# facebook/facebook360_dep

Measured on AMD Instinct MI355X. Metric: depth Mpix/s per GPU (full pyramid, 16-cam 2048^2 rig); % HBM-read roofline, higher is better.
Workload: dtype f32+f64; 1 GPU; BASELINE config 3: 16-camera 2048x2048 synthetic rig, 8-frame sequence, full 10-level pyramid per frame, per-level temporal filter (+-2 frames); the same sequence for every --gpus N (block partition, 8 frame(s) on this rank); rig=cfg2, cameras=16, frames=8, temporal_filter=True, halo_transport=local, parallelism=frames x1

## Files before the change

### facebook360_dep_amd/csrc/derp_capi.hip

```cpp
#include <hip/hip_runtime.h>

#include <algorithm>
#include <cmath>
#include <cstdarg>
#include <cstdio>
#include <cstdlib>
#include <cstring>
#include <map>
#include <memory>
#include <string>
#include <vector>

#include "../../include/derp_hip.h"
#include "derp_kernels.h"
#include "derp_points.h"
#include "derp_render.h"

using namespace derp;

namespace {

enum Stage {
  ST_FOV = 0,
  ST_VARIANCE,
// ... 1794 lines not shown
    return fail(c, "bad arguments");
  }
  const int L = c->cur;
  const size_t n = npx(c, L);
  TRY(upload_tmp(c, c->w.staging, disp, n));
  ALLOC(c, c->w.stagingB, 2 * n * sizeof(float));
  HIPCHK(c, hipMemsetAsync(c->w.stagingB.p, 0xff, 2 * n * sizeof(float), c->stream));
  LevelView V = make_view(c, ST_PINGPONG, 0, c->D);
  int tilesX;
  const int tiles = tiles_of(V.W, V.H, tilesX);
  const size_t lds = kCostLdsPerSrc * (size_t)(c->S);
  hipLaunchKernelGGL(k_cost_map, dim3(tiles), dim3(kCostBlock), lds, c->stream, V, d, c->w.staging.as<float>(),
                     c->w.stagingB.as<float>(), c->w.stagingB.as<float>() + n, tilesX);
  KCHECK(c);
  HIPCHK(c, hipStreamSynchronize(c->stream));
  HIPCHK(c, hipMemcpy(cost, c->w.stagingB.p, n * sizeof(float), hipMemcpyDeviceToHost));
  HIPCHK(c, hipMemcpy(confidence, c->w.stagingB.as<float>() + n, n * sizeof(float), hipMemcpyDeviceToHost));
  return 0;
}

int derp_debug_atan2_ypos(derp_ctx* c, const double* y, const double* x, double* out, size_t n) {
  if (!c || !y || !x || !out) {
    return fail(c, "bad arguments");
  }
  ALLOC(c, c->w.staging, 3 * n * sizeof(double));
  double* d = c->w.staging.as<double>();
  HIPCHK(c, hipMemcpyAsync(d, y, n * sizeof(double), hipMemcpyHostToDevice, c->stream));
  HIPCHK(c, hipMemcpyAsync(d + n, x, n * sizeof(double), hipMemcpyHostToDevice, c->stream));
  hipLaunchKernelGGL(k_debug_atan2_ypos, dim3(flat_grid(n)), dim3(256), 0, c->stream, d, d + n, d + 2 * n, n);
  KCHECK(c);
  HIPCHK(c, hipMemcpyAsync(out, d + 2 * n, n * sizeof(double), hipMemcpyDeviceToHost, c->stream));
  HIPCHK(c, hipStreamSynchronize(c->stream));
  return 0;
}

int derp_debug_fp64(derp_ctx* c, int op, const double* a, const double* b, double* out, size_t n) {
  if (!c || !a || !out || op < 0 || op > 3 || (op >= 2 && !b)) {
    return fail(c, "bad arguments");
  }
  if (n == 0) {
    return 0;
  }
  ALLOC(c, c->w.staging, 3 * n * sizeof(double));
  double* d = c->w.staging.as<double>();
  HIPCHK(c, hipMemcpyAsync(d, a, n * sizeof(double), hipMemcpyHostToDevice, c->stream));
  HIPCHK(c, hipMemcpyAsync(d + n, op >= 2 ? b : a, n * sizeof(double), hipMemcpyHostToDevice, c->stream));
  hipLaunchKernelGGL(k_debug_fp64, dim3(flat_grid(n)), dim3(256), 0, c->stream, op, d, d + n, d + 2 * n, n);
  KCHECK(c);
  HIPCHK(c, hipMemcpyAsync(out, d + 2 * n, n * sizeof(double), hipMemcpyDeviceToHost, c->stream));
  HIPCHK(c, hipStreamSynchronize(c->stream));
  return 0;
}

int derp_debug_sees(derp_ctx* c, int src, const double* xyz, size_t n, double* out) {
  if (!c || !xyz || !out || src < 0 || src >= c->S) {
    return fail(c, "bad arguments");
  }
  if (n == 0) {
    return 0;
  }
  ALLOC(c, c->w.staging, 9 * n * sizeof(double));
  double* d = c->w.staging.as<double>();
  HIPCHK(c, hipMemcpyAsync(d, xyz, 3 * n * sizeof(double), hipMemcpyHostToDevice, c->stream));
  hipLaunchKernelGGL(k_debug_sees, dim3(flat_grid(n)), dim3(256), 0, c->stream, c->camsSrc.as<Cam>(), src, d, d + 3 * n, n);
  KCHECK(c);
  HIPCHK(c, hipMemcpyAsync(out, d + 3 * n, 6 * n * sizeof(double), hipMemcpyDeviceToHost, c->stream));
  HIPCHK(c, hipStreamSynchronize(c->stream));
  return 0;
}

int derp_debug_download(derp_ctx* c, int d, int s, int which, void* out) {
  TRY(need_current(c, false));
  const int L = c->cur;
  const int W = c->LW[L], H = c->LH[L];
  const size_t n = (size_t)W * H;
  HIPCHK(c, hipStreamSynchronize(c->stream));
  if (which == 4) {
    HIPCHK(c, hipMemcpy(out, c->w.srcVar.as<float>() + (size_t)s * n, n * sizeof(float), hipMemcpyDeviceToHost));
    return 0;
  }
  if (which == 5) {
    HIPCHK(c, hipMemcpy(out, c->w.fovMask.as<uint8_t>() + (size_t)d * n, n, hipMemcpyDeviceToHost));
    return 0;
  }
  if (d < 0 || d >= c->D || s < 0 || s >= c->S || s == c->dst2srcH[d]) {
    return fail(c, "bad (dst, src) pair");
  }
  const size_t tab = (size_t)d * (c->S - 1) + (s < c->dst2srcH[d] ? s : s - 1);
  if (which == 0) {
    const int PW = W + 2 * kPadW, PH = H + 2 * kPadW;
    std::vector<float2> tmp((size_t)PW * PH);
    HIPCHK(c, hipMemcpy(tmp.data(), c->projWarp.as<float2>() + tab * tmp.size(), tmp.size() * sizeof(float2),
                        hipMemcpyDeviceToHost));
    float2* o = reinterpret_cast<float2*>(out);
    for (int y = 0; y < H; ++y) {
      memcpy(o + (size_t)y * W, &tmp[(size_t)(y + kPadW) * PW + kPadW], (size_t)W * sizeof(float2));
    }
    return 0;
  }
  if (which == 2 || which == 3) {
    const int PW = W + 2 * kPadC, PH = H + 2 * kPadC;
    std::vector<ushort4> tmp((size_t)PW * PH);
    const ushort4* base = (which == 2 ? c->w.projColor.as<ushort4>() : c->w.projBias.as<ushort4>()) + tab * tmp.size();
    HIPCHK(c, hipMemcpy(tmp.data(), base, tmp.size() * sizeof(ushort4), hipMemcpyDeviceToHost));
    uint16_t* o = reinterpret_cast<uint16_t*>(out);
    for (int y = 0; y < H; ++y) {
// ... 1060 lines not shown
```

### facebook360_dep_amd/csrc/derp_kernels.h

```cpp
#pragma once
#include <hip/hip_runtime.h>
#include <math.h>
#include <stdint.h>

#include <type_traits>

#include "derp_camera.h"
#include "gcc_algos.h"

namespace derp {

#ifndef DERP_COST_MIN_WAVES
#define DERP_COST_MIN_WAVES 4
#endif
#ifndef DERP_RANDOM_MIN_WAVES
#define DERP_RANDOM_MIN_WAVES 4
#endif
#ifndef DERP_RANDOM_TILED
#define DERP_RANDOM_TILED 0
#endif
#ifndef DERP_MIX_HOT_ONLY
#define DERP_MIX_HOT_ONLY 0
#endif
#ifndef DERP_PHASE_TIMERS
// ... 602 lines not shown
      const Cam& cs = V.camsSrc[s];
      D2 pn;
      const bool vis = sees<cost_sees_lean<RANDOM>()>(cs, pWorld, cs.principal[0], cs.principal[1], cs.focal[0], cs.focal[1],
                                                      1.0, 1.0, pn, pairs.atanLut);
      if (__ballot(pend) != 0ull) {
        consume();
      }
      pend = vis;
      pendSlot = slot(s, own);
      if (__ballot(vis) != 0ull) {
        const float sx = (float)(pn.x * V.Wd), sy = (float)(pn.y * V.Hd);
        const float xf = roundf(sx), yf = roundf(sy);
        const int xi = (int)xf, yi = (int)yf;
        pxw = sx - xf + 0.5f;
        pyw = sy - yf + 0.5f;
        const size_t tab = (size_t)dl * (V.S - 1) + pendSlot;
        const char* wbase = reinterpret_cast<const char*>(V.projWarp + tab * wPlane);
        const unsigned woff = vis ? ((unsigned)(yi - 1 + kPadW) * (unsigned)wPitch + (unsigned)(xi - 1 + kPadW)) * 8u : 0u;
        pa = *reinterpret_cast<const f4a8*>(wbase + woff);
        pb = *reinterpret_cast<const f4a8*>(wbase + (woff + (unsigned)wPitch * 8u));
      }
    }
    if (__ballot(pend) != 0ull) {
      consume();
    }
  }
  const unsigned tc1 = phase_clock();
  const int ssdCount = __popc(mask);
  nPair += ssdCount;
#ifdef DERP_COUNT_UNION
  if (slots) {
    *slots += __popc(__builtin_amdgcn_readfirstlane(waveMask));
  }
#endif
  int keep = 1;
  if (ssdCount < keep) {
    return make_float2(3.402823466e+38f, 0.0f);
  }
  {
    int cnt = 0;
    for (unsigned wm = __builtin_amdgcn_readfirstlane(waveMask); wm != 0; wm &= wm - 1) {
      const int t = __builtin_ctz(wm);
      if ((mask >> t) & 1) {
        const SsdPair e = pairs.get(t);
        const SsdPair ssd = compute_ssd<RANDOM>(V, px, colBase + (size_t)t * cPlane, biaBase + (size_t)t * cPlane, e.first,
                                                        e.second, RANDOM ? colTBase + (size_t)t * tPlane : nullptr);
        pairs.set(cnt, ssd);
        ++cnt;
      }
    }
  }
  const unsigned tc2 = phase_clock();
  keep = max(keep, ssdCount - 2);
  GccSelect<LdsPairs> sel(pairs);
  sel.nth_element(keep, ssdCount);
  float cost = 0;
  for (int i = 0; i < keep; ++i) {
    cost += pairs.get(i).second;
  }
  cost /= (float)keep;
  const float trustCoef = 1.0f / (float)keep;
  float confidence = px.confidence;
  if constexpr (RELOAD_RAY) {
    unsigned i = pix;
    asm("" : "+v"(i) : "v"(cost));
    if constexpr (RANDOM) {
      confidence = fmaxf(at32(V.srcVar + (size_t)own * ((size_t)V.W * V.H), i), kMinVar);
    } else {
      confidence = fmaxf((V.srcVar + (size_t)own * ((size_t)V.W * V.H))[i], kMinVar);
    }
  }
  const float costFinal = cost * trustCoef / confidence;
#if DERP_PHASE_TIMERS
  if (tm) {
    const unsigned tc3 = phase_clock();
    tm->proj += tc1 - tc0, tm->ssd += tc2 - tc1, tm->select += tc3 - tc2, tm->inside += tc3 - tc0;
  }
#endif
  return make_float2(costFinal, confidence);
}

template <bool WITH_RAY = true>
__device__ __forceinline__ void load_pixctx(const LevelView& V, int d, int own, int x, int y, const PatchWin* win, PixCtx& px,
                                            int tl = -1) {
  const Cam& cd = V.camsDst[d];
  px.rayO = {cd.pos[0], cd.pos[1], cd.pos[2]};
  const size_t n = (size_t)V.W * V.H;
  if constexpr (!WITH_RAY) {
    px.rayD = {0, 0, 0};
  } else {
    const size_t i = (size_t)d * n + (size_t)y * V.W + x;
    px.rayD = {V.rayDir[i], V.rayDir[V.rayStride + i], V.rayDir[2 * V.rayStride + i]};
  }
  if (tl < 0) {
    tl = (int)(threadIdx.x & 63);
  }
  const int corner = (tl >> 3) * kWinW + (tl & 7);
  px.winBG = win->bg + corner;
  px.winR = win->r + corner;
  const ushort4 b = V.ownBias[(size_t)own * n + (size_t)y * V.W + x];
  px.dstBiasBG = (v2f){(float)b.x, (float)b.y};
  px.dstBiasR = (float)b.z;
  const float var = V.srcVar[(size_t)own * n + (size_t)y * V.W + x];
  px.confidence = fmaxf(var, kMinVar);
}

__device__ __forceinline__ void flush_counters(const LevelView& V, unsigned nCost, unsigned nPair) {
  for (int off = 32; off > 0; off >>= 1) {
    nCost += __shfl_down(nCost, off);
    nPair += __shfl_down(nPair, off);
  }
  if ((threadIdx.x & 63) == 0) {
    atomicAdd(&V.counters[0], (unsigned long long)nCost);
    atomicAdd(&V.counters[1], (unsigned long long)nPair);
  }
}

__global__ void k_bgr_to_bgrx(const uint16_t* __restrict__ in, ushort4* __restrict__ out, size_t n) {
  size_t i = (size_t)blockIdx.x * blockDim.x + threadIdx.x;
  const size_t step = (size_t)gridDim.x * blockDim.x;
  for (; i < n; i += step) {
    out[i] = make_ushort4(in[3 * i], in[3 * i + 1], in[3 * i + 2], 0);
  }
}

__global__ void k_debug_atan2_ypos(const double* __restrict__ y, const double* __restrict__ x, double* __restrict__ out,
                                   size_t n) {
  size_t i = (size_t)blockIdx.x * blockDim.x + threadIdx.x;
  const size_t step = (size_t)gridDim.x * blockDim.x;
#if defined(__HIP_DEVICE_COMPILE__)
  __shared__ double atanLut[kAtanLutDoubles];
  atan_lut_fill(atanLut);
  __syncthreads();
  for (; i < n; i += step) {
    const double a = atan2_ypos(y[i], x[i]);
    const double b = atan2_ypos_lut(y[i], x[i], atanLut);
    out[i] = (__double_as_longlong(a) == __double_as_longlong(b)) ? b : __builtin_nan("");
  }
#endif
}

__global__ void k_debug_fp64(int op, const double* __restrict__ a, const double* __restrict__ b, double* __restrict__ out,
                             size_t n) {
  size_t i = (size_t)blockIdx.x * blockDim.x + threadIdx.x;
  const size_t step = (size_t)gridDim.x * blockDim.x;
#if defined(__HIP_DEVICE_COMPILE__)
  for (; i < n; i += step) {
    const double x = a[i], y = b[i];
    out[i] = op == 0 ? sqrt_lean(x) : op == 1 ? sqrt(x) : op == 2 ? div_plain(x, y) : x / y;
  }
#endif
}

__global__ void k_debug_sees(const Cam* __restrict__ cams, int src, const double* __restrict__ xyz, double* __restrict__ out,
                             size_t n) {
  size_t i = (size_t)blockIdx.x * blockDim.x + threadIdx.x;
  const size_t step = (size_t)gridDim.x * blockDim.x;
#if defined(__HIP_DEVICE_COMPILE__)
  __shared__ double atanLut[kAtanLutDoubles];
  atan_lut_fill(atanLut);
  __syncthreads();
  const Cam& cs = cams[src];
  for (; i < n; i += step) {
    const D3 p = {xyz[3 * i], xyz[3 * i + 1], xyz[3 * i + 2]};
    D2 a = {__builtin_nan(""), __builtin_nan("")}, b = a;
    const bool va = sees<cost_sees_lean<false>()>(cs, p, cs.principal[0], cs.principal[1], cs.focal[0], cs.focal[1], 1.0, 1.0,
                                                  a, atanLut);
    const bool vb = sees<cost_sees_lean<true>()>(cs, p, cs.principal[0], cs.principal[1], cs.focal[0], cs.focal[1], 1.0, 1.0,
                                                 b, atanLut);
    double* o = out + 6 * i;
    o[0] = va ? 1.0 : 0.0;
    o[1] = a.x;
    o[2] = a.y;
    o[3] = vb ? 1.0 : 0.0;
    o[4] = b.x;
    o[5] = b.y;
  }
#endif
}

__global__ void k_pixel_rays(LevelView V, double* __restrict__ rays, unsigned* __restrict__ behind) {
  const int d = V.dst0 + (int)blockIdx.z;
  const int x = blockIdx.x * blockDim.x + threadIdx.x, y = blockIdx.y * blockDim.y + threadIdx.y;
  if (x >= V.W || y >= V.H) {
    return;
  }
  const Cam& cd = V.camsDst[d];
  const D3 dir = rig_direction(cd, (x + 0.5) / (double)V.W, (y + 0.5) / (double)V.H, cd.principal[0], cd.principal[1],
                               cd.focal[0], cd.focal[1]);
  const size_t i = (size_t)d * ((size_t)V.W * V.H) + (size_t)y * V.W + x;
  rays[i] = dir.x;
  rays[V.rayStride + i] = dir.y;
  rays[2 * V.rayStride + i] = dir.z;
  behind[i] = behind_mask(V, V.dst2src[d], D3{cd.pos[0], cd.pos[1], cd.pos[2]}, dir);
}

__global__ void k_fov_mask(const Cam* __restrict__ cams, int W, int H, uint8_t* __restrict__ out) {
  const int d = blockIdx.z;
  const int x = blockIdx.x * blockDim.x + threadIdx.x, y = blockIdx.y * blockDim.y + threadIdx.y;
  if (x >= W || y >= H) {
    return;
  }
  const Cam& c = cams[d];
  const double px = (x + 0.5) / (double)W, py = (y + 0.5) / (double)H;
// ... 2191 lines not shown
```

### facebook360_dep_amd/csrc/gcc_algos.h

```cpp
#pragma once
#include <hip/hip_runtime.h>
#include <stdint.h>

#ifndef DERP_HD
#define DERP_HD __host__ __device__ __forceinline__
#endif

namespace derp {

struct alignas(8) SsdPair {
  float first, second;
};

DERP_HD unsigned long long pair_key(const SsdPair& a) {
  unsigned int hi, lo;
  __builtin_memcpy(&hi, &a.first, 4);
  __builtin_memcpy(&lo, &a.second, 4);
  return ((unsigned long long)hi << 32) | lo;
}
DERP_HD bool pair_less(const SsdPair& a, const SsdPair& b) {
  return pair_key(a) < pair_key(b);
}

template <typename A>
struct GccSelect {
  A& a;
  DERP_HD explicit GccSelect(A& acc) : a(acc) {}

  DERP_HD bool lt(int i, int j) {
    return pair_less(a.get(i), a.get(j));
  }
  DERP_HD void swap(int i, int j) {
    const SsdPair t = a.get(i);
    a.set(i, a.get(j));
    a.set(j, t);
  }

  DERP_HD unsigned long long move_median_to_first(int result, int ia, int ib, int ic) {
    const SsdPair pa = a.get(ia), pb = a.get(ib), pc = a.get(ic);
    const unsigned long long ka = pair_key(pa), kb = pair_key(pb), kc = pair_key(pc);
    int m;
    if (ka < kb) {
      m = (kb < kc) ? ib : (ka < kc) ? ic : ia;
    } else {
      m = (ka < kc) ? ia : (kb < kc) ? ic : ib;
    }
    const SsdPair pm = (m == ia) ? pa : (m == ib) ? pb : pc;
    const SsdPair pr = a.get(result);
    a.set(result, pm);
    a.set(m, pr);
    return pair_key(pm);
  }

  DERP_HD int unguarded_partition(int first, int last, unsigned long long kp) {
    for (;;) {
      SsdPair pf = a.get(first);
      while (pair_key(pf) < kp) {
        ++first;
        pf = a.get(first);
      }
      --last;
      SsdPair pl = a.get(last);
      while (kp < pair_key(pl)) {
        --last;
        pl = a.get(last);
      }
      if (!(first < last)) {
        return first;
      }
      a.set(first, pl);
      a.set(last, pf);
      ++first;
    }
  }

  DERP_HD int unguarded_partition_pivot(int first, int last) {
    const int mid = first + (last - first) / 2;
    const unsigned long long kp = move_median_to_first(first, first + 1, mid, last - 1);
    return unguarded_partition(first + 1, last, kp);
  }

  DERP_HD void insertion_sort(int first, int last) {
    if (first == last) {
      return;
    }
    for (int i = first + 1; i != last; ++i) {
      const SsdPair val = a.get(i);
      if (pair_less(val, a.get(first))) {
        for (int k = i; k > first; --k) {
          a.set(k, a.get(k - 1));
        }
        a.set(first, val);
      } else {
        int hole = i;
        int next = i - 1;
        while (pair_less(val, a.get(next))) {
          a.set(hole, a.get(next));
          hole = next;
          --next;
        }
        a.set(hole, val);
      }
    }
  }

  DERP_HD void push_heap(int first, int hole, int top, const SsdPair& value) {
    int parent = (hole - 1) / 2;
    while (hole > top && pair_less(a.get(first + parent), value)) {
      a.set(first + hole, a.get(first + parent));
      hole = parent;
      parent = (hole - 1) / 2;
    }
    a.set(first + hole, value);
  }
  DERP_HD void adjust_heap(int first, int hole, int len, const SsdPair& value) {
    const int top = hole;
    int child = hole;
    while (child < (len - 1) / 2) {
      child = 2 * (child + 1);
      if (lt(first + child, first + (child - 1))) {
        child--;
      }
      a.set(first + hole, a.get(first + child));
      hole = child;
    }
    if ((len & 1) == 0 && child == (len - 2) / 2) {
      child = 2 * (child + 1);
      a.set(first + hole, a.get(first + (child - 1)));
      hole = child - 1;
    }
    push_heap(first, hole, top, value);
  }
  DERP_HD void make_heap(int first, int last) {
    const int len = last - first;
    if (len < 2) {
      return;
    }
    int parent = (len - 2) / 2;
    for (;;) {
      const SsdPair value = a.get(first + parent);
      adjust_heap(first, parent, len, value);
      if (parent == 0) {
        return;
      }
      parent--;
    }
  }
  DERP_HD void heap_select(int first, int middle, int last) {
    make_heap(first, middle);
    for (int i = middle; i < last; ++i) {
      if (lt(i, first)) {
        const SsdPair value = a.get(i);
        a.set(i, a.get(first));
        adjust_heap(first, 0, middle - first, value);
      }
    }
  }

  DERP_HD void nth_element(int nth, int n) {
    int first = 0, last = n;
    if (first == last || nth == last) {
      return;
    }
    int depth_limit = 2 * (31 - __builtin_clz((unsigned)n));
    while (last - first > 3) {
      if (depth_limit == 0) {
        heap_select(first, nth + 1, last);
        swap(first, nth);
        return;
      }
      --depth_limit;
      const int cut = unguarded_partition_pivot(first, last);
      if (cut <= nth) {
        first = cut;
      } else {
        last = cut;
      }
    }
    insertion_sort3(first, last);
  }

  DERP_HD void insertion_sort3(int first, int last) {
    const int cnt = last - first;
    if (cnt < 2) {
      return;
    }
    SsdPair p0 = a.get(first), p1 = a.get(first + 1);
    if (pair_key(p1) < pair_key(p0)) {
      const SsdPair t = p0;
      p0 = p1;
      p1 = t;
    }
    if (cnt == 3) {
      const SsdPair p2 = a.get(first + 2);
      const unsigned long long k2 = pair_key(p2);
      if (k2 < pair_key(p0)) {
        a.set(first + 2, p1);
        p1 = p0;
        p0 = p2;
      } else if (k2 < pair_key(p1)) {
        a.set(first + 2, p1);
        p1 = p2;
      }
    }
    a.set(first, p0);
    a.set(first + 1, p1);
  }
};

static constexpr uint32_t kMinstdA = 16807u;
static constexpr uint32_t kMinstdM = 2147483647u;

DERP_HD uint32_t minstd_mulmod(uint32_t x, uint32_t y) {
  const uint64_t p = (uint64_t)x * (uint64_t)y;
  uint64_t t = (p & kMinstdM) + (p >> 31);
  t = (t & kMinstdM) + (t >> 31);
  return (uint32_t)(t >= kMinstdM ? t - kMinstdM : t);
}
DERP_HD uint32_t minstd_seed(int s) {
  const uint32_t v = (uint32_t)((uint64_t)(uint32_t)s % kMinstdM);
  return v == 0 ? 1u : v;
}
DERP_HD uint32_t minstd_jump(uint32_t state, uint64_t n) {
  uint32_t mult = 1u, base = kMinstdA;
  while (n) {
    if (n & 1) {
      mult = minstd_mulmod(mult, base);
    }
    base = minstd_mulmod(base, base);
    n >>= 1;
  }
  return minstd_mulmod(state, mult);
}
DERP_HD float minstd_uniform(uint32_t& state, float a, float b) {
  state = minstd_mulmod(state, kMinstdA);
  float u = (float)(state - 1u) / 2147483648.0f;
  if (u >= 1.0f) {
    u = 0.99999994f;
  }
  return u * (b - a) + a;
}

}
```

### facebook360_dep_amd/derp.py

```python
import ctypes as C
import os

import numpy as np

_HERE = os.path.dirname(os.path.abspath(__file__))
LIB_PATH = os.environ.get("DERP_LIB") or os.path.join(_HERE, "libderp_hip.so")
CAM_TYPES = {"FTHETA": 0, "RECTILINEAR": 1, "EQUISOLID": 2, "ORTHOGRAPHIC": 3}

STAGES = ["fov_mask", "variance", "own_bias", "upsample", "proj_warp", "reproject", "proj_bias", "brute_force",
          "random_proposals", "ping_pong", "mismatches", "bilateral", "median", "mask_fov", "temporal"]


class SeqOptions(C.Structure):
    _fields_ = [
        ("time_radius", C.c_int32), ("sigma", C.c_float), ("weight_b", C.c_float), ("weight_g", C.c_float),
        ("weight_r", C.c_float), ("space_radius", C.c_int32), ("use_foreground_masks", C.c_int32),
        ("partition", C.c_int32), ("do_temporal_filter", C.c_int32), ("resident_frames", C.c_int32),
    ]


class SeqTransfer(C.Structure):
    _fields_ = [("frame", C.c_int32), ("from_rank", C.c_int32), ("to_rank", C.c_int32)]


# ... 14 lines not shown
        ("use_foreground_masks", C.c_int32), ("partial_coverage", C.c_int32), ("rebuild_warp_tables", C.c_int32),
    ]


class RenderParams(C.Structure):
    _fields_ = [
        ("kind", C.c_int32), ("width", C.c_int32), ("height", C.c_int32), ("position", C.c_double * 3),
        ("forward", C.c_double * 3), ("up", C.c_double * 3), ("horizontal_fov", C.c_double), ("ipd", C.c_float),
        ("alpha_blend", C.c_int32), ("disparity_color", C.c_int32), ("weight", C.c_int32), ("zero_nans", C.c_int32),
    ]


RENDER_KINDS = {"cube": 0, "equirect": 1, "snapshot": 2}
WEIGHTS = {"svd": 0, "minor": 1}
FORMATS = ["cubecolor", "cubedisp", "eqrcolor", "eqrdisp", "lr180", "snapcolor", "snapdisp", "tb3dof", "tbstereo"]


def render_params(kind="equirect", width=3072, height=None, position=(0, 0, 0), forward=(-1, 0, 0), up=(0, 0, 1),
                  horizontal_fov=90.0, ipd=0.0, alpha_blend=True, disparity_color=False, weight="svd", zero_nans=False):
    p = RenderParams()
    lib().derp_render_params_default(C.byref(p))
    p.kind = RENDER_KINDS[kind]
    p.width = width
    p.height = width // 2 if height is None else height
    for k, v in (("position", position), ("forward", forward), ("up", up)):
        for i in range(3):
            getattr(p, k)[i] = float(v[i])
    p.horizontal_fov = horizontal_fov
    p.ipd = ipd
    p.alpha_blend = int(bool(alpha_blend))
    p.disparity_color = int(bool(disparity_color))
    p.weight = WEIGHTS[weight]
    p.zero_nans = int(bool(zero_nans))
    return p


def render_format_size(fmt, width, height):
    w, h = C.c_int(), C.c_int()
    if lib().derp_render_format_size(fmt.encode(), width, height, C.byref(w), C.byref(h)):
        raise ValueError("Invalid format: %s" % fmt)
    return w.value, h.value


EXPORTS = [
    "derp_options_default", "derp_create", "derp_destroy", "derp_last_error", "derp_set_options", "derp_set_pyramid",
    "derp_build_pyramid_color", "derp_build_pyramid_foreground_mask", "derp_build_pyramid_background_disparity",
    "derp_download_level_color", "derp_download_level_mask", "derp_download_level_background", "derp_resize_area",
    "derp_generate_foreground_mask", "derp_image_info", "derp_image_decode", "derp_image_last_error", "derp_jpeg_encode",
    "derp_upload_color", "derp_upload_foreground_mask", "derp_upload_background_disparity", "derp_upload_disparity",
    "derp_process_level", "derp_process_pyramid", "derp_synchronize", "derp_download_disparity", "derp_download_cost",
    "derp_level_begin", "derp_stage_reproject_colors", "derp_stage_brute_force", "derp_stage_random_proposals",
    "derp_stage_ping_pong", "derp_stage_mismatches", "derp_stage_bilateral_filter", "derp_stage_median_filter", "derp_stage_mask_fov",
    "derp_level_end", "derp_set_level_disparity", "derp_get_level_disparity", "derp_cost_map", "derp_debug_download",
    "derp_debug_atan2_ypos", "derp_debug_fp64", "derp_debug_sees",
    "derp_ssim", "derp_average_score", "derp_rephotograph", "derp_rephotograph_upload", "derp_rephotograph_render", "derp_canopy_cubemap",
    "derp_render_params_default", "derp_render_upload", "derp_render", "derp_render_format_size", "derp_render_format",
    "derp_render_vertices",
    "derp_export_points", "derp_points_begin", "derp_points_splat", "derp_points_download", "derp_project_equirect_mask",
    "derp_fov_mask", "derp_layer_disparities", "derp_download_mismatch_mask", "derp_upsample_disparity", "derp_joint_bilateral_u16", "derp_joint_bilateral_f32", "derp_masked_median",
    "derp_temporal_filter", "derp_temporal_filter_dev", "derp_dev_disparity", "derp_dev_color", "derp_dev_mask",
    "derp_get_counters", "derp_reset_counters", "derp_profile_enable", "derp_profile_reset", "derp_profile_query", "derp_profile_memoised",
    "derp_device_name", "derp_device_memory", "derp_host_nth_element_pairs", "derp_host_minstd_uniform",
    "derp_set_frame_slots", "derp_select_frame", "derp_frame_slots", "derp_host_alloc", "derp_host_free", "derp_bind_thread", "derp_host_register", "derp_host_unregister",
    "derp_seq_options_default", "derp_seq_window", "derp_seq_owner", "derp_seq_plan", "derp_seq_create", "derp_seq_destroy",
    "derp_seq_counts", "derp_seq_frames", "derp_seq_frame_slot", "derp_seq_buffer", "derp_rccl_unique_id",
    "derp_seq_attach_rccl", "derp_seq_attach_loopback", "derp_seq_attach_external", "derp_seq_selftest",
    "derp_seq_exchange_inputs", "derp_seq_level_compute", "derp_seq_level_exchange", "derp_seq_level_filter",
    "derp_seq_host_inputs", "derp_seq_buffer_copy", "derp_seq_upload_color_plane", "derp_seq_upload_disparity", "derp_seq_download_disparity", "derp_seq_exchange_inputs_level",
    "derp_seq_level_compute_frame", "derp_seq_level_provided_frame", "derp_seq_mark_exchanged", "derp_seq_level_filter_frame", "derp_seq_download_filtered",
    "derp_seq_run", "derp_seq_stats", "derp_seq_stats_reset", "derp_seq_exchange_exposed_ms",
]

_lib = None


def lib():
    global _lib
    if _lib is None:
        if not os.path.exists(LIB_PATH):
            raise RuntimeError(
                "libderp_hip.so is missing: build it with `python -c 'import __graft_entry__ as g; g.build()'` "
                "(hipcc --offload-arch=gfx950). There is no CPU fallback for the depth path."
            )
        try:
            import torch
        except ImportError:
            pass
        _lib = C.CDLL(LIB_PATH)
        _lib.derp_last_error.restype = C.c_char_p
        _lib.derp_last_error.argtypes = [C.c_void_p]
        _lib.derp_host_minstd_uniform.restype = C.c_float
        _lib.derp_host_minstd_uniform.argtypes = [C.c_int, C.c_uint64, C.c_float, C.c_float]
    return _lib


def camera_desc(cam):
    j = CameraDesc()
    j.type = CAM_TYPES[cam["type"]]
    for k in ("origin", "forward", "up", "right", "resolution", "focal"):
        for i, v in enumerate(cam[k]):
            getattr(j, k)[i] = float(v)
    j.has_principal = int("principal" in cam)
    if "principal" in cam:
        j.principal[0], j.principal[1] = map(float, cam["principal"])
    j.has_distortion = int("distortion" in cam)
    if "distortion" in cam:
        d = list(cam["distortion"]) + [0.0] * (3 - len(cam["distortion"]))
# ... 192 lines not shown

    def level_begin(self, level):
        self._cur = level
        self._ck(lib().derp_level_begin(self.h, level))

    def stage(self, name):
        fn = {
            "reproject_colors": "derp_stage_reproject_colors", "brute_force": "derp_stage_brute_force",
            "random_proposals": "derp_stage_random_proposals", "ping_pong": "derp_stage_ping_pong",
            "mismatches": "derp_stage_mismatches", "bilateral": "derp_stage_bilateral_filter", "median": "derp_stage_median_filter",
            "mask_fov": "derp_stage_mask_fov", "end": "derp_level_end",
        }[name]
        self._ck(getattr(lib(), fn)(self.h))

    def set_level_disparity(self, d, disp):
        disp = np.ascontiguousarray(disp, dtype=np.float32)
        self._ck(lib().derp_set_level_disparity(self.h, d, _p(disp)))

    def get_level_disparity(self, d):
        out = np.zeros(self._shape(self._cur), dtype=np.float32)
        self._ck(lib().derp_get_level_disparity(self.h, d, _p(out)))
        return out

    def cost_map(self, d, disp):
        disp = np.ascontiguousarray(disp, dtype=np.float32)
        cost = np.zeros(self._shape(self._cur), dtype=np.float32)
        conf = np.zeros(self._shape(self._cur), dtype=np.float32)
        self._ck(lib().derp_cost_map(self.h, d, _p(disp), _p(cost), _p(conf)))
        return cost, conf

    def debug_atan2_ypos(self, y, x):
        y = np.ascontiguousarray(y, np.float64)
        x = np.ascontiguousarray(x, np.float64)
        out = np.zeros_like(y)
        self._ck(lib().derp_debug_atan2_ypos(self.h, _p(y), _p(x), _p(out), C.c_size_t(y.size)))
        return out

    FP64_OPS = {"sqrt_lean": 0, "sqrt": 1, "div_plain": 2, "div": 3}

    def debug_fp64(self, op, a, b=None):
        a = np.ascontiguousarray(a, np.float64)
        b = None if b is None else np.ascontiguousarray(b, np.float64)
        assert b is None or b.shape == a.shape
        out = np.zeros_like(a)
        self._ck(lib().derp_debug_fp64(self.h, self.FP64_OPS[op], _p(a), _p(b), _p(out), C.c_size_t(a.size)))
        return out

    def debug_sees(self, src, xyz):
        xyz = np.ascontiguousarray(xyz, np.float64).reshape(-1, 3)
        out = np.zeros((len(xyz), 2, 3))
        self._ck(lib().derp_debug_sees(self.h, src, _p(xyz), C.c_size_t(len(xyz)), _p(out)))
        return out[:, :, 0].T != 0, np.ascontiguousarray(out[:, :, 1:].transpose(1, 0, 2))

    def debug(self, d, s, which):
        h, w = self._shape(self._cur)
        spec = {"warp": (0, (h, w, 2), np.float32), "color": (2, (h, w, 3), np.uint16),
                "bias": (3, (h, w, 3), np.uint16), "variance": (4, (h, w), np.float32),
                "fov": (5, (h, w), np.uint8)}[which]
        out = np.zeros(spec[1], dtype=spec[2])
        self._ck(lib().derp_debug_download(self.h, d, s, spec[0], _p(out)))
        return out

    def mismatch_mask(self, d):
        out = np.zeros(self._shape(self._cur), dtype=np.uint8)
        self._ck(lib().derp_download_mismatch_mask(self.h, d, _p(out)))
        return out

    def layer_disparities(self, fg, bg):
        fg = np.ascontiguousarray(fg, dtype=np.float32)
        bg = np.ascontiguousarray(bg, dtype=np.float32)
        out = np.zeros(fg.shape, dtype=np.uint8)
        self._ck(lib().derp_layer_disparities(self.h, _p(fg), _p(bg), C.c_size_t(fg.size), _p(out)))
        return out

    def ssim(self, x, y, blur_radius=1, alpha=1.0, beta=1.0, gamma=1.0):
        x = np.ascontiguousarray(x, dtype=np.float32)
        y = np.ascontiguousarray(y, dtype=np.float32)
        h, w = x.shape[:2]
        out = np.zeros((h, w, 3), dtype=np.float32)
        self._ck(lib().derp_ssim(self.h, _p(x), _p(y), w, h, blur_radius, C.c_float(alpha), C.c_float(beta),
                                 C.c_float(gamma), _p(out)))
        return out

    def rephotograph(self, target, colors, disps):
        colors = [np.ascontiguousarray(c, dtype=np.uint16) for c in colors]
        disps = [np.ascontiguousarray(d, dtype=np.float32) for d in disps]
        h, w = disps[0].shape
        cp = (C.c_void_p * len(colors))(*[c.ctypes.data for c in colors])
        dp = (C.c_void_p * len(disps))(*[d.ctypes.data for d in disps])
        out = np.zeros((h, w, 4), dtype=np.float32)
        self._ck(lib().derp_rephotograph(self.h, target, cp, dp, w, h, _p(out)))
        return out

    def rephotograph_upload(self, colors, disps):
        colors = [np.ascontiguousarray(c, dtype=np.uint16) for c in colors]
        disps = [np.ascontiguousarray(d, dtype=np.float32) for d in disps]
        h, w = disps[0].shape
        cp = (C.c_void_p * len(colors))(*[c.ctypes.data for c in colors])
        dp = (C.c_void_p * len(disps))(*[d.ctypes.data for d in disps])
        self._ck(lib().derp_rephotograph_upload(self.h, cp, dp, w, h))

    def canopy_cubemap(self, include, centre, edge):
        inc = np.ascontiguousarray(include, dtype=np.uint8)
        ctr = np.ascontiguousarray(centre, dtype=np.float64)
        out = np.zeros((6 * edge, edge, 4), dtype=np.float32)
        self._ck(lib().derp_canopy_cubemap(self.h, _p(inc), _p(ctr), edge, _p(out)))
# ... 226 lines not shown
```

### include/derp_hip.h

```cpp
#ifndef DERP_HIP_H
#define DERP_HIP_H

#include <stddef.h>
#include <stdint.h>

#ifdef __cplusplus
extern "C" {
#endif

typedef struct derp_ctx derp_ctx;

enum { DERP_FTHETA = 0, DERP_RECTILINEAR = 1, DERP_EQUISOLID = 2, DERP_ORTHOGRAPHIC = 3 };

typedef struct {
  int32_t type;
  int32_t has_principal;
  int32_t has_distortion;
  int32_t has_fov;
  double origin[3];
  double forward[3];
  double up[3];
  double right[3];
  double resolution[2];
  double focal[2];
// ... 36 lines not shown
void* derp_host_alloc(size_t bytes);
void derp_host_free(void* p);
int derp_bind_thread(derp_ctx* ctx);
int derp_host_register(void* p, size_t bytes);
void derp_host_unregister(void* p);

int derp_upload_color(derp_ctx* ctx, int level, int src, const uint16_t* bgr);
int derp_upload_foreground_mask(derp_ctx* ctx, int level, int src, const uint8_t* mask);
int derp_upload_background_disparity(derp_ctx* ctx, int level, int dst, const float* disp);
int derp_upload_disparity(derp_ctx* ctx, int level, int dst, const float* disp);

int derp_build_pyramid_color(derp_ctx* ctx, int src, const uint16_t* bgr, int w, int h);
int derp_build_pyramid_foreground_mask(derp_ctx* ctx, int src, const uint8_t* mask, int w, int h,
                                       int threshold);
int derp_build_pyramid_background_disparity(derp_ctx* ctx, int dst, const float* disp, int w, int h);
int derp_download_level_color(derp_ctx* ctx, int level, int src, uint16_t* bgr);
int derp_download_level_mask(derp_ctx* ctx, int level, int src, uint8_t* mask01);
int derp_download_level_background(derp_ctx* ctx, int level, int dst, float* disp);
int derp_image_info(const void* bytes, size_t n, int* w, int* h, int* channels, int* bitdepth);
int derp_image_decode(const void* bytes, size_t n, void* out, size_t out_bytes);
const char* derp_image_last_error(void);
int derp_jpeg_encode(const void* pixels, int w, int h, int channels, int quality, void* out, size_t cap, size_t* size);

int derp_resize_area(derp_ctx* ctx, int kind, const void* src, int w, int h, void* dst, int dw, int dh);

int derp_generate_foreground_mask(derp_ctx* ctx, const uint16_t* template_bgr, const uint16_t* frame_bgr,
                                  int w, int h, int blur_radius, float threshold,
                                  int morph_closing_size, uint8_t* mask01);

int derp_process_level(derp_ctx* ctx, int level);
int derp_process_pyramid(derp_ctx* ctx, int level_start, int level_end);
int derp_synchronize(derp_ctx* ctx);

int derp_download_disparity(derp_ctx* ctx, int level, int dst, float* disparity);
int derp_download_cost(derp_ctx* ctx, int dst, float* cost, float* confidence);

int derp_level_begin(derp_ctx* ctx, int level);
int derp_stage_reproject_colors(derp_ctx* ctx);
int derp_stage_brute_force(derp_ctx* ctx);
int derp_stage_random_proposals(derp_ctx* ctx);
int derp_stage_ping_pong(derp_ctx* ctx);
int derp_stage_mismatches(derp_ctx* ctx);
int derp_stage_bilateral_filter(derp_ctx* ctx);
int derp_stage_median_filter(derp_ctx* ctx);
int derp_stage_mask_fov(derp_ctx* ctx);
int derp_level_end(derp_ctx* ctx);
int derp_set_level_disparity(derp_ctx* ctx, int dst, const float* disp);
int derp_get_level_disparity(derp_ctx* ctx, int dst, float* disp);
int derp_cost_map(derp_ctx* ctx, int dst, const float* disp, float* cost, float* confidence);
int derp_debug_download(derp_ctx* ctx, int dst, int src, int which, void* out);
int derp_debug_atan2_ypos(derp_ctx* ctx, const double* y, const double* x, double* out, size_t n);
int derp_debug_fp64(derp_ctx* ctx, int op, const double* a, const double* b, double* out, size_t n);
int derp_debug_sees(derp_ctx* ctx, int src, const double* xyz, size_t n, double* out);

int derp_download_mismatch_mask(derp_ctx* ctx, int dst, uint8_t* out);

int derp_layer_disparities(derp_ctx* ctx, const float* foreground, const float* background, size_t n,
                           uint8_t* out);
int derp_ssim(derp_ctx* ctx, const float* x_bgr, const float* y_bgr, int w, int h, int blur_radius, float alpha,
              float beta, float gamma, float* score_bgr);
int derp_average_score(const float* score_bgr, const uint8_t* mask, int w, int h, double* avg_bgr3);
int derp_rephotograph(derp_ctx* ctx, int target, const uint16_t* const* colors, const float* const* disparities,
                      int w, int h, float* out_bgra);
int derp_rephotograph_upload(derp_ctx* ctx, const uint16_t* const* colors, const float* const* disparities, int w,
                             int h);
int derp_rephotograph_render(derp_ctx* ctx, int target, float* out_bgra);
int derp_canopy_cubemap(derp_ctx* ctx, const uint8_t* include, const double* centre, int edge, float* out_bgra);
enum { DERP_RENDER_CUBE = 0, DERP_RENDER_EQUIRECT = 1, DERP_RENDER_SNAPSHOT = 2 };
enum { DERP_WEIGHT_SVD = 0, DERP_WEIGHT_MINOR = 1 };
typedef struct {
  int32_t kind;
  int32_t width, height;
  double position[3];
  double forward[3], up[3];
  double horizontal_fov;
  float ipd;
  int32_t alpha_blend;
  int32_t disparity_color;
  int32_t weight;
  int32_t zero_nans;
} derp_render_params;
void derp_render_params_default(derp_render_params* p);
int derp_render_upload(derp_ctx* ctx, const float* const* colors_bgra, const int* color_w, const int* color_h,
                       const float* const* disparities, const int* disp_w, const int* disp_h);
int derp_render(derp_ctx* ctx, const derp_render_params* p, const uint8_t* include, float* out_bgra);
int derp_render_format_size(const char* format, int width, int height, int* out_w, int* out_h);
int derp_render_format(derp_ctx* ctx, const char* format, const derp_render_params* p, const float* background,
                       const float* background_equirect, int eq_w, int eq_h, float* out_bgra);
int derp_render_vertices(derp_ctx* ctx, int cam, float ipd, float* out_xyzw);
int derp_export_points(derp_ctx* ctx, int cam, const float* disparity, int w, int h, const float* color_bgr,
                       double max_depth, int clip, int subsample, float* out_xyzrgb, size_t cap, size_t* count);
int derp_points_begin(derp_ctx* ctx, const int* widths, const int* heights);
int derp_points_splat(derp_ctx* ctx, const double* xyz, size_t n, double min_depth, double max_depth);
int derp_points_download(derp_ctx* ctx, int cam, float* disparity);
int derp_project_equirect_mask(derp_ctx* ctx, int cam, const uint8_t* eqr, int eqr_w, int eqr_h, int w, int h,
                               double depth, uint8_t* out);
int derp_fov_mask(derp_ctx* ctx, int dst, int w, int h, uint8_t* out);
int derp_upsample_disparity(derp_ctx* ctx, int dst, const float* disp, int w, int h,
                            const float* bg_disp_up, const uint8_t* fg_mask,
                            const uint8_t* fg_mask_up, int w_up, int h_up,
                            int use_foreground_masks, float* out);
int derp_joint_bilateral_u16(derp_ctx* ctx, const float* image, const uint16_t* guide_bgr,
                             const uint8_t* mask, int w, int h, int radius, float sigma,
                             float weight0, float weight1, float weight2, float* out);
int derp_joint_bilateral_f32(derp_ctx* ctx, const float* image, const float* guide_bgr,
                             const uint8_t* mask, int w, int h, int radius, float sigma,
// ... 88 lines not shown
```

Baseline: 475.9 Mpix/s.

## Replace LDS nth_element with register rank-based permutation select for small n

For pixels with at most 8 SSD candidates, the cost selection now computes pairwise ranks of 64-bit keys in registers and runs a quickselect over a packed 4-bit permutation word, instead of swapping pairs in LDS. A fallback through a permutation view keeps the original GCC nth_element ordering when NaN-like keys are present, and larger n still uses the LDS path. The aim is to cut LDS traffic and divergent branching in the per-pixel select, at the cost of more registers and an O(n^2) rank computation. A debug kernel and API entry are added to check the new selection.

```diff
diff --git a/facebook360_dep_amd/csrc/derp_capi.hip b/facebook360_dep_amd/csrc/derp_capi.hip
--- a/facebook360_dep_amd/csrc/derp_capi.hip
+++ b/facebook360_dep_amd/csrc/derp_capi.hip
@@ -1870,6 +1870,31 @@
   return 0;
 }
 
+int derp_debug_select(derp_ctx* c, const float* rows, size_t lanes, float* out, uint32_t* perm) {
+  if (!c || !rows || !out || !perm) {
+    return fail(c, "bad arguments");
+  }
+  for (size_t l = 0; l < lanes; ++l) {
+    if (!(rows[32 * l] >= 1.0f && rows[32 * l] <= (float)(kDebugSelectSlots - 1))) {
+      return fail(c, "derp_debug_select: n must lie in 1..15");
+    }
+  }
+  if (lanes == 0) {
+    return 0;
+  }
+  ALLOC(c, c->w.staging, lanes * (64 * sizeof(float) + sizeof(uint32_t)));
+  float* d = c->w.staging.as<float>();
+  uint32_t* dp = reinterpret_cast<uint32_t*>(d + 64 * lanes);
+  HIPCHK(c, hipMemcpyAsync(d, rows, lanes * 32 * sizeof(float), hipMemcpyHostToDevice, c->stream));
+  hipLaunchKernelGGL(k_debug_select, dim3((unsigned)((lanes + 63) / 64)), dim3(64), kDebugSelectSlots * 64 * sizeof(SsdPair),
+                     c->stream, d, d + 32 * lanes, dp, (int)lanes);
+  KCHECK(c);
+  HIPCHK(c, hipMemcpyAsync(out, d + 32 * lanes, lanes * 32 * sizeof(float), hipMemcpyDeviceToHost, c->stream));
+  HIPCHK(c, hipMemcpyAsync(perm, dp, lanes * sizeof(uint32_t), hipMemcpyDeviceToHost, c->stream));
+  HIPCHK(c, hipStreamSynchronize(c->stream));
+  return 0;
+}
+
 int derp_debug_sees(derp_ctx* c, int src, const double* xyz, size_t n, double* out) {
   if (!c || !xyz || !out || src < 0 || src >= c->S) {
     return fail(c, "bad arguments");
diff --git a/facebook360_dep_amd/csrc/derp_kernels.h b/facebook360_dep_amd/csrc/derp_kernels.h
--- a/facebook360_dep_amd/csrc/derp_kernels.h
+++ b/facebook360_dep_amd/csrc/derp_kernels.h
@@ -678,12 +678,7 @@
   }
   const unsigned tc2 = phase_clock();
   keep = max(keep, ssdCount - 2);
-  GccSelect<LdsPairs> sel(pairs);
-  sel.nth_element(keep, ssdCount);
-  float cost = 0;
-  for (int i = 0; i < keep; ++i) {
-    cost += pairs.get(i).second;
-  }
+  float cost = select_sum(pairs, keep, ssdCount);
   cost /= (float)keep;
   const float trustCoef = 1.0f / (float)keep;
   float confidence = px.confidence;
@@ -776,6 +771,36 @@
     out[i] = op == 0 ? sqrt_lean(x) : op == 1 ? sqrt(x) : op == 2 ? div_plain(x, y) : x / y;
   }
 #endif
+}
+
+static constexpr int kDebugSelectSlots = 16;
+__global__ void __launch_bounds__(64)
+    k_debug_select(const float* __restrict__ rows, float* __restrict__ out, unsigned* __restrict__ perms, int lanes) {
+  extern __shared__ SsdPair ldsPairs[];
+  const int l = (int)(blockIdx.x * 64 + threadIdx.x);
+  if (l >= lanes) {
+    return;
+  }
+  LdsPairs pairs{ldsPairs + threadIdx.x, 64, nullptr};
+  const float* row = rows + (size_t)32 * l;
+  const int n = min(max((int)row[0], 1), kDebugSelectSlots - 1);
+  for (int i = 0; i < n; ++i) {
+    pairs.set(i, SsdPair{row[2 + 2 * i], row[3 + 2 * i]});
+  }
+  unsigned perm;
+  const float sum = select_sum(pairs, max(1, n - 2), n, &perm);
+  float* o = out + (size_t)32 * l;
+  o[0] = sum;
+  o[1] = 0.f;
+  for (int i = 0; i < n; ++i) {
+    const SsdPair p = pairs.get(n <= kSelectSmallN ? (int)perm_field(perm, 4 * i) : i);
+    o[2 + 2 * i] = p.first;
+    o[3 + 2 * i] = p.second;
+  }
+  for (int i = 2 + 2 * n; i < 32; ++i) {
+    o[i] = 0.f;
+  }
+  perms[l] = perm;
 }
 
 __global__ void k_debug_sees(const Cam* __restrict__ cams, int src, const double* __restrict__ xyz, double* __restrict__ out,
diff --git a/facebook360_dep_amd/csrc/gcc_algos.h b/facebook360_dep_amd/csrc/gcc_algos.h
--- a/facebook360_dep_amd/csrc/gcc_algos.h
+++ b/facebook360_dep_amd/csrc/gcc_algos.h
@@ -1,5 +1,7 @@
 #pragma once
+#if defined(__HIP__) || defined(__HIPCC__)
 #include <hip/hip_runtime.h>
+#endif
 #include <stdint.h>
 
 #ifndef DERP_HD
@@ -22,46 +24,59 @@
   return pair_key(a) < pair_key(b);
 }
 
-template <typename A>
+struct PairKeyLess {
+  static DERP_HD bool lt(const SsdPair& a, const SsdPair& b) {
+    return pair_key(a) < pair_key(b);
+  }
+};
+struct PairFloatLess {
+  static DERP_HD bool lt(const SsdPair& a, const SsdPair& b) {
+    return a.first < b.first || (!(b.first < a.first) && a.second < b.second);
+  }
+};
+
+template <typename A, typename Less = PairKeyLess>
 struct GccSelect {
   A& a;
+  template <typename U>
+  static U& ref_of();
+  using T = decltype(ref_of<A>().get(0));
   DERP_HD explicit GccSelect(A& acc) : a(acc) {}
 
   DERP_HD bool lt(int i, int j) {
-    return pair_less(a.get(i), a.get(j));
+    return Less::lt(a.get(i), a.get(j));
   }
   DERP_HD void swap(int i, int j) {
-    const SsdPair t = a.get(i);
+    const T t = a.get(i);
     a.set(i, a.get(j));
     a.set(j, t);
   }
 
-  DERP_HD unsigned long long move_median_to_first(int result, int ia, int ib, int ic) {
-    const SsdPair pa = a.get(ia), pb = a.get(ib), pc = a.get(ic);
-    const unsigned long long ka = pair_key(pa), kb = pair_key(pb), kc = pair_key(pc);
+  DERP_HD T move_median_to_first(int result, int ia, int ib, int ic) {
+    const T pa = a.get(ia), pb = a.get(ib), pc = a.get(ic);
     int m;
-    if (ka < kb) {
-      m = (kb < kc) ? ib : (ka < kc) ? ic : ia;
+    if (Less::lt(pa, pb)) {
+      m = Less::lt(pb, pc) ? ib : Less::lt(pa, pc) ? ic : ia;
     } else {
-      m = (ka < kc) ? ia : (kb < kc) ? ic : ib;
-    }
-    const SsdPair pm = (m == ia) ? pa : (m == ib) ? pb : pc;
-    const SsdPair pr = a.get(result);
+      m = Less::lt(pa, pc) ? ia : Less::lt(pb, pc) ? ic : ib;
+    }
+    const T pm = (m == ia) ? pa : (m == ib) ? pb : pc;
+    const T pr = a.get(result);
     a.set(result, pm);
     a.set(m, pr);
-    return pair_key(pm);
-  }
-
-  DERP_HD int unguarded_partition(int first, int last, unsigned long long kp) {
+    return pm;
+  }
+
+  DERP_HD int unguarded_partition(int first, int last, const T& pv) {
     for (;;) {
-      SsdPair pf = a.get(first);
-      while (pair_key(pf) < kp) {
+      T pf = a.get(first);
+      while (Less::lt(pf, pv)) {
         ++first;
         pf = a.get(first);
       }
       --last;
-      SsdPair pl = a.get(last);
-      while (kp < pair_key(pl)) {
+      T pl = a.get(last);
+      while (Less::lt(pv, pl)) {
         --last;
         pl = a.get(last);
       }
@@ -76,8 +91,8 @@
 
   DERP_HD int unguarded_partition_pivot(int first, int last) {
     const int mid = first + (last - first) / 2;
-    const unsigned long long kp = move_median_to_first(first, first + 1, mid, last - 1);
-    return unguarded_partition(first + 1, last, kp);
+    const T pv = move_median_to_first(first, first + 1, mid, last - 1);
+    return unguarded_partition(first + 1, last, pv);
   }
 
   DERP_HD void insertion_sort(int first, int last) {
@@ -85,8 +100,8 @@
       return;
     }
     for (int i = first + 1; i != last; ++i) {
-      const SsdPair val = a.get(i);
-      if (pair_less(val, a.get(first))) {
+      const T val = a.get(i);
+      if (Less::lt(val, a.get(first))) {
         for (int k = i; k > first; --k) {
           a.set(k, a.get(k - 1));
         }
@@ -94,7 +109,7 @@
       } else {
         int hole = i;
         int next = i - 1;
-        while (pair_less(val, a.get(next))) {
+        while (Less::lt(val, a.get(next))) {
           a.set(hole, a.get(next));
           hole = next;
           --next;
@@ -104,16 +119,16 @@
     }
   }
 
-  DERP_HD void push_heap(int first, int hole, int top, const SsdPair& value) {
+  DERP_HD void push_heap(int first, int hole, int top, const T& value) {
     int parent = (hole - 1) / 2;
-    while (hole > top && pair_less(a.get(first + parent), value)) {
+    while (hole > top && Less::lt(a.get(first + parent), value)) {
       a.set(first + hole, a.get(first + parent));
       hole = parent;
       parent = (hole - 1) / 2;
     }
     a.set(first + hole, value);
   }
-  DERP_HD void adjust_heap(int first, int hole, int len, const SsdPair& value) {
+  DERP_HD void adjust_heap(int first, int hole, int len, const T& value) {
     const int top = hole;
     int child = hole;
     while (child < (len - 1) / 2) {
@@ -138,7 +153,7 @@
     }
     int parent = (len - 2) / 2;
     for (;;) {
-      const SsdPair value = a.get(first + parent);
+      const T value = a.get(first + parent);
       adjust_heap(first, parent, len, value);
       if (parent == 0) {
         return;
@@ -150,7 +165,7 @@
     make_heap(first, middle);
     for (int i = middle; i < last; ++i) {
       if (lt(i, first)) {
-        const SsdPair value = a.get(i);
+        const T value = a.get(i);
         a.set(i, a.get(first));
         adjust_heap(first, 0, middle - first, value);
       }
@@ -185,20 +200,19 @@
     if (cnt < 2) {
       return;
     }
-    SsdPair p0 = a.get(first), p1 = a.get(first + 1);
-    if (pair_key(p1) < pair_key(p0)) {
-      const SsdPair t = p0;
+    T p0 = a.get(first), p1 = a.get(first + 1);
+    if (Less::lt(p1, p0)) {
+      const T t = p0;
       p0 = p1;
       p1 = t;
     }
     if (cnt == 3) {
-      const SsdPair p2 = a.get(first + 2);
-      const unsigned long long k2 = pair_key(p2);
-      if (k2 < pair_key(p0)) {
+      const T p2 = a.get(first + 2);
+      if (Less::lt(p2, p0)) {
         a.set(first + 2, p1);
         p1 = p0;
         p0 = p2;
-      } else if (k2 < pair_key(p1)) {
+      } else if (Less::lt(p2, p1)) {
         a.set(first + 2, p1);
         p1 = p2;
       }
@@ -207,6 +221,155 @@
     a.set(first + 1, p1);
   }
 };
+
+static constexpr int kSelectSmallN = 8;
+static constexpr unsigned kPermIdentity = 0x76543210u;
+
+DERP_HD bool wave_any(bool c) {
+#if defined(__HIP_DEVICE_COMPILE__)
+  return __ballot(c) != 0ull;
+#else
+  return c;
+#endif
+}
+
+struct TaggedPair : SsdPair {
+  unsigned id;
+};
+template <typename A>
+struct PermView {
+  A& a;
+  unsigned perm;
+  DERP_HD TaggedPair get(int i) const {
+    TaggedPair t;
+    t.id = (perm >> (4 * i)) & 15u;
+    const SsdPair p = a.get((int)t.id);
+    t.first = p.first;
+    t.second = p.second;
+    return t;
+  }
+  DERP_HD void set(int i, const TaggedPair& v) {
+    perm = (perm & ~(15u << (4 * i))) | (v.id << (4 * i));
+  }
+};
+
+DERP_HD void perm_swap(unsigned& w, int p4, int q4, bool c = true) {
+  unsigned x = ((w >> p4) ^ (w >> q4)) & 15u;
+  x = c ? x : 0u;
+  w ^= (x << p4) | (x << q4);
+}
+DERP_HD unsigned perm_field(unsigned w, int p4) {
+  return (w >> p4) & 15u;
+}
+
+template <typename A>
+DERP_HD unsigned select_small_perm(A& a, int keep, int n) {
+  unsigned long long k[kSelectSmallN];
+  unsigned top = 0;
+#pragma unroll
+  for (int j = 0; j < kSelectSmallN; ++j) {
+    k[j] = ~0ull;
+    if (wave_any(j < n)) {
+      if (j < n) {
+        const SsdPair p = a.get(j);
+        k[j] = pair_key(p);
+        const unsigned hi = (unsigned)(k[j] >> 32), lo = (unsigned)k[j];
+        top = top > hi ? top : hi;
+        top = top > lo ? top : lo;
+      }
+    }
+  }
+  if (top > 0x7f800000u) {
+    PermView<A> view{a, kPermIdentity};
+    GccSelect<PermView<A>, PairFloatLess> sel(view);
+    sel.nth_element(keep, n);
+    return view.perm;
+  }
+  unsigned rank = 0;
+#pragma unroll
+  for (int j = 0; j < kSelectSmallN; ++j) {
+    if (wave_any(j < n)) {
+      unsigned below = 0;
+#pragma unroll
+      for (int i = 0; i < kSelectSmallN; ++i) {
+        if (i != j) {
+          below += k[i] < k[j] ? 1u : 0u;
+        }
+      }
+      rank |= below << (4 * j);
+    }
+  }
+  unsigned perm = kPermIdentity;
+  constexpr unsigned kHigh = 0x88888888u, kOnes = 0x11111111u;
+  int first4 = 0, last4 = 4 * n;
+  const int nth4 = 4 * keep;
+  while (last4 - first4 > 12) {
+    const int a4 = first4 + 4, b4 = first4 + (((last4 - first4) >> 3) << 2), c4 = last4 - 4;
+    const unsigned ra = perm_field(rank, a4), rb = perm_field(rank, b4), rc = perm_field(rank, c4);
+    int m4;
+    if (ra < rb) {
+      m4 = (rb < rc) ? b4 : (ra < rc) ? c4 : a4;
+    } else {
+      m4 = (ra < rc) ? a4 : (rb < rc) ? c4 : b4;
+    }
+    perm_swap(perm, first4, m4);
+    perm_swap(rank, first4, m4);
+    const unsigned pivot = perm_field(rank, first4) * kOnes;
+    int f4 = first4 + 4, l4 = last4;
+    for (;;) {
+      const unsigned ge = ((rank | kHigh) - pivot) & kHigh;
+      const unsigned le = ((pivot | kHigh) - rank) & kHigh;
+      f4 += __builtin_ctz((ge >> f4) | 0x80000000u) & ~3;
+      l4 -= 4 + __builtin_clz((le << (32 - l4)) | 1u);
+      if (!(f4 < l4)) {
+        break;
+      }
+      perm_swap(perm, f4, l4);
+      perm_swap(rank, f4, l4);
+      f4 += 4;
+    }
+    if (f4 <= nth4) {
+      first4 = f4;
+    } else {
+      last4 = f4;
+    }
+  }
+  const int cnt4 = last4 - first4;
+  const int p1 = (first4 + 4) & 28, p2 = (first4 + 8) & 28;
+  unsigned r0 = perm_field(rank, first4), r1 = perm_field(rank, p1);
+  const unsigned r2 = perm_field(rank, p2);
+  const bool s01 = cnt4 >= 8 && r1 < r0;
+  perm_swap(perm, first4, p1, s01);
+  if (s01) {
+    const unsigned t = r0;
+    r0 = r1;
+    r1 = t;
+  }
+  const bool s12 = cnt4 == 12 && r2 < r1;
+  perm_swap(perm, p1, p2, s12);
+  perm_swap(perm, first4, p1, s12 && r2 < r0);
+  return perm;
+}
+
+template <typename A>
+DERP_HD float select_sum(A& a, int keep, int n, unsigned* permOut = nullptr) {
+  unsigned perm = kPermIdentity;
+  if (n > kSelectSmallN) {
+    GccSelect<A> sel(a);
+    sel.nth_element(keep, n);
+  } else {
+    perm = select_small_perm(a, keep, n);
+  }
+  float sum = 0;
+  for (int i = 0; i < keep; ++i) {
+    const int at = n > kSelectSmallN ? i : (int)perm_field(perm, (4 * i) & 31);
+    sum += a.get(at).second;
+  }
+  if (permOut) {
+    *permOut = perm;
+  }
+  return sum;
+}
 
 static constexpr uint32_t kMinstdA = 16807u;
 static constexpr uint32_t kMinstdM = 2147483647u;
diff --git a/facebook360_dep_amd/derp.py b/facebook360_dep_amd/derp.py
--- a/facebook360_dep_amd/derp.py
+++ b/facebook360_dep_amd/derp.py
@@ -90,7 +90,7 @@
     "derp_level_begin", "derp_stage_reproject_colors", "derp_stage_brute_force", "derp_stage_random_proposals",
     "derp_stage_ping_pong", "derp_stage_mismatches", "derp_stage_bilateral_filter", "derp_stage_median_filter", "derp_stage_mask_fov",
     "derp_level_end", "derp_set_level_disparity", "derp_get_level_disparity", "derp_cost_map", "derp_debug_download",
-    "derp_debug_atan2_ypos", "derp_debug_fp64", "derp_debug_sees",
+    "derp_debug_atan2_ypos", "derp_debug_fp64", "derp_debug_sees", "derp_debug_select",
     "derp_ssim", "derp_average_score", "derp_rephotograph", "derp_rephotograph_upload", "derp_rephotograph_render", "derp_canopy_cubemap",
     "derp_render_params_default", "derp_render_upload", "derp_render", "derp_render_format_size", "derp_render_format",
     "derp_render_vertices",
@@ -389,6 +389,13 @@
         self._ck(lib().derp_debug_sees(self.h, src, _p(xyz), C.c_size_t(len(xyz)), _p(out)))
         return out[:, :, 0].T != 0, np.ascontiguousarray(out[:, :, 1:].transpose(1, 0, 2))
 
+    def debug_select(self, rows):
+        rows = np.ascontiguousarray(rows, np.float32).reshape(-1, 32)
+        out = np.zeros_like(rows)
+        perm = np.zeros(len(rows), dtype=np.uint32)
+        self._ck(lib().derp_debug_select(self.h, _p(rows), C.c_size_t(len(rows)), _p(out), _p(perm)))
+        return out[:, 0].copy(), out[:, 2:].reshape(-1, 15, 2).copy(), perm
+
     def debug(self, d, s, which):
         h, w = self._shape(self._cur)
         spec = {"warp": (0, (h, w, 2), np.float32), "color": (2, (h, w, 3), np.uint16),
diff --git a/include/derp_hip.h b/include/derp_hip.h
--- a/include/derp_hip.h
+++ b/include/derp_hip.h
@@ -112,6 +112,7 @@
 int derp_debug_atan2_ypos(derp_ctx* ctx, const double* y, const double* x, double* out, size_t n);
 int derp_debug_fp64(derp_ctx* ctx, int op, const double* a, const double* b, double* out, size_t n);
 int derp_debug_sees(derp_ctx* ctx, int src, const double* xyz, size_t n, double* out);
+int derp_debug_select(derp_ctx* ctx, const float* rows, size_t lanes, float* out, uint32_t* perm);
 
 int derp_download_mismatch_mask(derp_ctx* ctx, int dst, uint8_t* out);
 
```

Measured after the change: 479.6 Mpix/s (median of 6 runs). Within noise of the previous version (+0.8%).
